# HandBrake/HandBrake

Measured on AMD Instinct MI355X. Metric: filtered frames/sec, 1080p YUV420p NLMeans+decomb chain, higher is better.
Workload: dtype u8 (f32 NLMeans weights, 16-bit fixed-point scaler as zimg, sharpen mix = the reference's f64 expression, as one f32 multiply where init proves that equal); 1 GPU; BASELINE configs[3]: decomb(31, EEDI2 bob) -> nlmeans medium -> cropscale lanczos 1920x1080 -> 3840x2160 -> lapsharp, 1080i YUV420P 8-bit in, inputs resident in HBM; input=1920x1080, output=3840x2160, streams_per_gpu=1, content=interlaced, stream_frames=48, stage_streams=2, parallelism=1 GPU(s) x 1 independent stream(s), device=AMD Radeon Graphics (gfx950:sramecc+:xnack-, 256 CUs)

## Files before the change

### handbrake_amd/csrc/eedi2.hip

```cpp
#include "eedi2_vote.h"
#include "eedi2_engine.h"

#include <atomic>
#include <algorithm>

namespace {

constexpr int PEAK = 255, NEUTRAL = 128;
constexpr int EEDI_MAX_FIELDS = EEDI_MAX_BATCH;
constexpr size_t GUARD = 32768;

__constant__ uint8_t c_limlut[33] = { 6, 6, 7, 7, 8, 8, 9, 9, 9, 10, 10, 11, 11, 12, 12, 12, 12, 12, 12, 12,
                                      12, 12, 12, 12, 12, 12, 12, 12, 12, 12, 12, 255, 255 };

constexpr int LIM_N = 33, LIM_PAD = 40;
__device__ __forceinline__ void lim_fill(uint8_t *tab, int tid)
{
    if (tid < LIM_N) tab[tid] = c_limlut[tid];
}

struct P3
{
    uint8_t *a[3];
    uint8_t *b[3];
    uint8_t *c[3];
    uint8_t *d[3];
    uint8_t *e[3];
    uint8_t *f[3];
    uint8_t *g[3];
    int pitch[3], width[3], height[3];
    size_t   fstride;
    uint32_t tffbits;
    const uint32_t *pflags;
    uint32_t pepoch;
};

struct PL { uint8_t *a, *b, *c, *d, *e, *f, *g; };
__device__ __forceinline__ PL plane_ptrs(const P3 &P, int pl, size_t off)
{
    PL q = { P.a[pl] + off, P.b[pl] + off, P.c[pl] + off, P.d[pl], P.e[pl] + off, P.f[pl] + off, P.g[pl] + off };
    if (q.d) q.d += off;
    return q;
}
#define FIELD_PLANE(P)                                                      \
    const int fld = (int)blockIdx.z / 3, pl = (int)blockIdx.z - 3 * fld;    \
    const int tff = (int)(((P).tffbits >> fld) & 1u);                       \
    const PL Q = plane_ptrs((P), pl, (size_t)fld * (P).fstride);            \
     \
     \
    const bool maskless = (P).pflags[blockIdx.z] != (P).pepoch;             \
    (void)tff; (void)maskless

__device__ __forceinline__ int iabs(int v) { return v < 0 ? -v : v; }
__device__ __forceinline__ int hbhip_align_up_dev(int v, int a) { return (v + a - 1) / a * a; }

__device__ __forceinline__ int wave_list_slots(int *counter, unsigned n)
{
    const uint64_t b0 = __ballot(n & 1u), b1 = __ballot(n & 2u), b2 = __ballot(n & 4u);
    const int total = __popcll(b0) + 2 * __popcll(b1) + 4 * __popcll(b2);
    auto below = [](uint64_t m) { return (int)__builtin_amdgcn_mbcnt_hi((uint32_t)(m >> 32), __builtin_amdgcn_mbcnt_lo((uint32_t)m, 0u)); };
    int base = 0;
    if (total)
    {
        if ((threadIdx.x & 63) == 0) base = atomicAdd(counter, total);
        base = __builtin_amdgcn_readfirstlane(base);
    }
    return base + below(b0) + 2 * below(b1) + 4 * below(b2);
}

__device__ __forceinline__ int sad3(const uint8_t *a, int ai, const uint8_t *b, int bi)
{
    return iabs((int)a[ai - 1] - (int)b[bi - 1]) + iabs((int)a[ai] - (int)b[bi]) + iabs((int)a[ai + 1] - (int)b[bi + 1]);
}

__device__ __forceinline__ int sorted_mid(int *v, int n)
{
    for (int i = 1; i < n; i++)
    {
        const int t = v[i];
        int j = i;
        while (j > 0 && v[j - 1] > t) { v[j] = v[j - 1]; j--; }
        v[j] = t;
    }
    return (n & 1) ? v[n >> 1] : (v[(n - 1) >> 1] + v[n >> 1] + 1) >> 1;
}


constexpr int ABSENT = 1000;

__device__ __forceinline__ void cswap(int &a, int &b)
{
    const int lo = min(a, b), hi = max(a, b);
    a = lo; b = hi;
}

__device__ __forceinline__ int mid9(int &v0, int &v1, int &v2, int &v3, int &v4, int &v5, int &v6, int &v7, int &v8, int n)
{
    cswap(v0, v3); cswap(v1, v7); cswap(v2, v5); cswap(v4, v8);
    cswap(v0, v7); cswap(v2, v4); cswap(v3, v8); cswap(v5, v6);
    cswap(v0, v2); cswap(v1, v3); cswap(v4, v5); cswap(v7, v8);
    cswap(v1, v4); cswap(v3, v6); cswap(v5, v7);
    cswap(v0, v1); cswap(v2, v4); cswap(v3, v5); cswap(v6, v8);
    cswap(v2, v3); cswap(v4, v5); cswap(v6, v7);
    cswap(v1, v2); cswap(v3, v4); cswap(v5, v6);
    const bool n5 = n <= 5, n7 = n <= 7;
    const int hi = n5 ? v2 : (n7 ? v3 : v4);
    const int lo = n5 ? v1 : (n7 ? v2 : v3);
    return (n & 1) ? hi : (lo + hi + 1) >> 1;
}

__device__ __forceinline__ int mid6(int &v0, int &v1, int &v2, int &v3, int &v4, int &v5, int n)
{
    cswap(v0, v5); cswap(v1, v3); cswap(v2, v4);
    cswap(v1, v2); cswap(v3, v4);
    cswap(v0, v3); cswap(v2, v5);
    cswap(v0, v1); cswap(v2, v3); cswap(v4, v5);
    cswap(v1, v2); cswap(v3, v4);
    const int lo = n <= 4 ? v1 : v2;
    const int hi = n <= 3 ? v1 : (n <= 5 ? v2 : v3);
    return (n & 1) ? hi : (lo + hi + 1) >> 1;
}

__device__ __forceinline__ void vote1(int v, int mid, int lim, int &sum, int &cnt)
{
    const bool in = (int)__builtin_amdgcn_sad_u16((uint32_t)v, (uint32_t)mid, 0u) <= lim;
    cnt += in;
    sum += in ? v : 0;
}

#define XY_PLANE(P)                                                         \
    FIELD_PLANE(P);                                                         \
    const int x = blockIdx.x * blockDim.x + threadIdx.x;                    \
    const int y = blockIdx.y * blockDim.y + threadIdx.y;                    \
    const int pitch = (P).pitch[pl], width = (P).width[pl], height = (P).height[pl]; \
    (void)width; (void)height; (void)pitch

struct Win12 { uint32_t w0, w1, w2; };

__device__ __forceinline__ Win12 ldwin(const uint8_t *row_at_x)
{
    const uint32_t *p = reinterpret_cast<const uint32_t *>(row_at_x);
    return Win12{p[-1], p[0], p[1]};
}

__device__ __forceinline__ int wb(const Win12 &w, int i)
{
    const int k = i + 4;
    const uint32_t d = k < 4 ? w.w0 : (k < 8 ? w.w1 : w.w2);
    return (int)((d >> (8 * (k & 3))) & 0xffu);
}

__device__ __forceinline__ void st4(uint8_t *dst_at_x, const int (&out)[4], int x, int limit)
{
// ... 367 lines not shown
        if (!(y == 1 || mp[x - 1 + u] == PEAK || mp[x + u] == PEAK || mp[x + 1 + u] == PEAK)) continue;
        if (!(y == height - 2 || mn[x - 1 - u] == PEAK || mn[x - u] == PEAK || mn[x + 1 - u] == PEAK)) continue;
        const int diffsn = sad3(sc, x, sn, x - u);
        const int diffsp = sad3(sc, x, sp, x + u);
        const int diffps = sad3(sp, x, sc, x - u);
        const int diffns = sad3(sn, x, sc, x + u);
        const int diff = diffsn + diffsp + diffps + diffns;
        int diffd = diffsp + diffns, diffe = diffsn + diffps;
        if (diff < minb) { dirb = u; minb = diff; }
        if (y > 1)
        {
            const int diff2pp = sad3(s2p, x, sp, x - u);
            const int diffp2p = sad3(sp, x, s2p, x + u);
            const int diffa = diff + diff2pp + diffp2p;
            diffd += diffp2p;
            diffe += diff2pp;
            if (diffa < mina) { dira = u; mina = diffa; }
        }
        if (y < height - 2)
        {
            const int diff2nn = sad3(s2n, x, sn, x + u);
            const int diffn2n = sad3(sn, x, s2n, x - u);
            const int diffc = diff + diff2nn + diffn2n;
            diffd += diff2nn;
            diffe += diffn2n;
            if (diffc < minc) { dirc = u; minc = diffc; }
        }
        if (diffd < mind) { dird = u; mind = diffd; }
        if (diffe < mine) { dire = u; mine = diffe; }
    }
    int order[5], k = 0;
    if (dira != -5000) order[k++] = dira;
    if (dirb != -5000) order[k++] = dirb;
    if (dirc != -5000) order[k++] = dirc;
    if (dird != -5000) order[k++] = dird;
    if (dire != -5000) order[k++] = dire;
    int out = NEUTRAL;
    if (k > 1)
    {
        const int mid = sorted_mid(order, k);
        const int tlim = max((int)c_limlut[iabs(mid)] >> 2, 2);
        int sum = 0, cnt = 0;
        for (int i = 0; i < k; i++)
            if (iabs(order[i] - mid) <= tlim) { cnt++; sum += order[i]; }
        if (cnt > 1) out = (NEUTRAL + ((int)((float)sum / (float)cnt) * 4)) & 0xff;
    }
    Q.c[(size_t)y * pitch + x] = (uint8_t)out;
}

#ifdef HBHIP_DEV_STATS
__device__ unsigned long long g_cd_stats[24];
#define CD_STAT(i, v) atomicAdd(&g_cd_stats[i], (unsigned long long)(v))
#else
#define CD_STAT(i, v) ((void)0)
#endif
constexpr int CD_W = 256, CD_HALO = 32, CD_LW = CD_W + 2 * CD_HALO;



__device__ __forceinline__ int calc_dir_vote(int ta, int tb, int tc, int td, int te)
{
    constexpr int BIG = 1 << 20;
    int v0 = ta ? ta - 32 : BIG, v1 = tb ? tb - 32 : BIG, v2 = tc ? tc - 32 : BIG, v3 = td ? td - 32 : BIG, v4 = te ? te - 32 : BIG;
    const int k = (ta != 0) + (tb != 0) + (tc != 0) + (td != 0) + (te != 0);
#define CD_CX(a, b) { const int lo_ = min(a, b), hi_ = max(a, b); a = lo_; b = hi_; }
    CD_CX(v0, v1) CD_CX(v3, v4) CD_CX(v2, v4) CD_CX(v2, v3) CD_CX(v0, v3) CD_CX(v0, v2) CD_CX(v1, v4) CD_CX(v1, v3) CD_CX(v1, v2)
#undef CD_CX
    int out = NEUTRAL;
    if (k > 1)
    {
        const int lo = k == 2 ? v0 : (k == 5 ? v2 : v1);
        const int hi = k >= 4 ? v2 : v1;
        const int mid = (lo + hi + 1) >> 1;
        static_assert(CD_HALO - 2 <= 30, "the closed form of limlut covers entries 0..30");
        const int tlim = iabs(mid) >= 13 ? 3 : 2;
        int sum = 0, cnt = 0;
        if (iabs(v0 - mid) <= tlim) { cnt++; sum += v0; }
        if (iabs(v1 - mid) <= tlim) { cnt++; sum += v1; }
        if (iabs(v2 - mid) <= tlim) { cnt++; sum += v2; }
        if (iabs(v3 - mid) <= tlim) { cnt++; sum += v3; }
        if (iabs(v4 - mid) <= tlim) { cnt++; sum += v4; }
        if (cnt > 1) out = (NEUTRAL + ((int)((float)sum / (float)cnt) * 4)) & 0xff;
    }
    return out;
}

template <bool EDGE, typename PASS>
__device__ __forceinline__ int calc_dir_search(const uint32_t *tr, PASS pass, int maxdt, bool first, bool last, int nt13, int nt19)
{
    const uint32_t F2p = tr[0], Fp = tr[CD_LW], Fc = tr[2 * CD_LW], Fn = tr[3 * CD_LW], F2n = tr[4 * CD_LW];
    const int ctr = (int)((Fc >> 8) & 0xff);
    const int vert = iabs(ctr - (int)((Fn >> 8) & 0xff)) + iabs(ctr - (int)((Fp >> 8) & 0xff));
    uint32_t kb = (uint32_t)min(nt13, vert * 6) << 16, ka = (uint32_t)min(nt19, vert * 9) << 16;
    uint32_t kc = ka, kd = kb, ke = kb;
    typedef __attribute__((address_space(3))) const uint32_t *lds_u32;
    uint32_t ap0 = (uint32_t)(uintptr_t)(lds_u32)(tr - maxdt), am0 = (uint32_t)(uintptr_t)(lds_u32)(tr + maxdt);
    uint32_t tag0 = (uint32_t)(32 - maxdt);
    asm volatile("" : "+v"(ap0), "+v"(am0), "+s"(tag0));
#define SADH(a, b, acc) __builtin_amdgcn_sad_hi_u8((a), (b), (acc))
    while (pass)
    {
        const int jj = sizeof(PASS) == 8 ? __ffsll((unsigned long long)pass) - 1 : __ffs((unsigned int)pass) - 1;
        pass &= pass - (PASS)1;
        const uint32_t tag = (uint32_t)jj + tag0;
        const lds_u32 tp = (lds_u32)(uintptr_t)(ap0 + 4u * (uint32_t)jj), tm = (lds_u32)(uintptr_t)(am0 - 4u * (uint32_t)jj);
        const uint32_t e1 = SADH(Fp, tm[2 * CD_LW], SADH(Fc, tm[3 * CD_LW], 0u));
        const uint32_t d1 = SADH(Fn, tp[2 * CD_LW], SADH(Fc, tp[1 * CD_LW], tag));
        const uint32_t diff = e1 + d1;
        uint32_t diffd = d1, diffe = e1;
        kb = min(kb, diff);
        if (!EDGE || !first)
        {
            const uint32_t diff2pp = SADH(F2p, tm[1 * CD_LW], tag);
            const uint32_t diffp2p = SADH(Fp, tp[0 * CD_LW], 0u);
            diffd += diffp2p;
            diffe += diff2pp;
            ka = min(ka, diff + diff2pp + diffp2p);
        }
        else
            diffe += tag;
        if (!EDGE || !last)
        {
            const uint32_t diff2nn = SADH(F2n, tp[3 * CD_LW], 0u);
            const uint32_t diffn2n = SADH(Fn, tm[4 * CD_LW], 0u);
            diffd += diff2nn;
            diffe += diffn2n;
            kc = min(kc, diff + diff2nn + diffn2n);
        }
        kd = min(kd, diffd);
        ke = min(ke, diffe);
    }
#undef SADH
    return calc_dir_vote((int)((ka & 0xffffu) >> 1), (int)(kb & 0xffffu), (int)(kc & 0xffffu), (int)(kd & 0xffffu), (int)(ke & 0xffffu));
}

template <int R, bool PRED>
__device__ __forceinline__ void calc_dir_dense(const uint32_t *tr, int maxdt, const uint32_t (&up)[R], const uint32_t (&dn)[R],
                                               int nt13, int nt19, uint32_t (&ka)[R], uint32_t (&kb)[R], uint32_t (&kc)[R],
                                               uint32_t (&kd)[R], uint32_t (&ke)[R])
{
    constexpr int NS = R + 4, NE = R + 3;
#define SADH(a, b, acc) __builtin_amdgcn_sad_hi_u8((a), (b), (acc))
    uint32_t T[NS];
#pragma unroll
    for (int r = 0; r < NS; r++) T[r] = tr[r * CD_LW];
#pragma unroll
    for (int j = 0; j < R; j++)
    {
        const int ctr = (int)((T[j + 2] >> 8) & 0xff);
        const int vert = iabs(ctr - (int)((T[j + 3] >> 8) & 0xff)) + iabs(ctr - (int)((T[j + 1] >> 8) & 0xff));
        kb[j] = (uint32_t)min(nt13, vert * 6) << 16; ka[j] = (uint32_t)min(nt19, vert * 9) << 16;
        kc[j] = ka[j]; kd[j] = kb[j]; ke[j] = kb[j];
    }
    auto sums = [&](const uint32_t (&Pv)[NE], const uint32_t (&Qv)[NE], const uint32_t (&X)[R], uint32_t (&ca)[R], uint32_t (&cb)[R],
                    uint32_t (&cc)[R], uint32_t (&cd)[R], uint32_t (&ce)[R]) {
        uint32_t S[NE], P2[NE - 1], Q2[NE - 1];
#pragma unroll
        for (int r = 0; r < NE; r++) S[r] = Pv[r] + Qv[r];
#pragma unroll
        for (int r = 0; r < NE - 1; r++) { P2[r] = Pv[r] + Pv[r + 1]; Q2[r] = Qv[r] + Qv[r + 1]; }
        if (PRED)
        {
#pragma unroll
            for (int j = 0; j < R; j++)
            {
                cb[j] = S[j + 1] + S[j + 2] + X[j]; ca[j] = cb[j] + S[j]; cc[j] = cb[j] + S[j + 3];
                ce[j] = P2[j] + P2[j + 2] + X[j];   cd[j] = Q2[j] + Q2[j + 2] + X[j];
            }
        }
        else
        {
            uint32_t S2[NE - 1], S3[NE - 2];
#pragma unroll
            for (int r = 0; r < NE - 1; r++) S2[r] = S[r] + S[r + 1];
#pragma unroll
            for (int r = 0; r < NE - 2; r++) S3[r] = S2[r] + S[r + 2];
#pragma unroll
            for (int j = 0; j < R; j++)
            {
                cb[j] = S2[j + 1]; ca[j] = S3[j]; cc[j] = S3[j + 1];
                ce[j] = P2[j] + P2[j + 2]; cd[j] = Q2[j] + Q2[j + 2];
            }
        }
    };
    uint32_t X1[R], X2[R];
#pragma unroll
    for (int j = 0; j < R; j++) { X1[j] = 0; X2[j] = 0; }
    {
        uint32_t Pv[NE], ca[R], cb[R], cc[R], cd[R], ce[R];
#pragma unroll
        for (int r = 0; r < NE; r++) Pv[r] = SADH(T[r], T[r + 1], 32u);
        if (PRED)
        {
#pragma unroll
            for (int j = 0; j < R; j++) X1[j] = (up[j] << 30) & 0x40000000u;
        }
        sums(Pv, Pv, X1, ca, cb, cc, cd, ce);
#pragma unroll
        for (int j = 0; j < R; j++)
        {
            ka[j] = min(ka[j], ca[j]); kb[j] = min(kb[j], cb[j]); kc[j] = min(kc[j], cc[j]);
            kd[j] = min(kd[j], cd[j]); ke[j] = min(ke[j], ce[j]);
        }
    }
    for (int d = 1; d <= maxdt; d++)
    {
        const uint32_t *tp = tr + d, *tm = tr - d;
        uint32_t Pl[NS], Mi[NS];
#pragma unroll
        for (int r = 0; r < NS; r++) { Pl[r] = tp[r * CD_LW]; Mi[r] = tm[r * CD_LW]; }
        const uint32_t t1 = 32u + (uint32_t)d, t2 = 32u - (uint32_t)d;
        uint32_t P1[NE], Q1[NE], Pn[NE], Qn[NE];
#pragma unroll
        for (int r = 0; r < NE; r++)
        {
            P1[r] = SADH(T[r], Mi[r + 1], t1); Q1[r] = SADH(Pl[r], T[r + 1], t1);
            Pn[r] = SADH(T[r], Pl[r + 1], t2); Qn[r] = SADH(Mi[r], T[r + 1], t2);
        }
        if (PRED)
        {
            const uint32_t sh = 30u - (uint32_t)d;
#pragma unroll
            for (int j = 0; j < R; j++) { X1[j] = (up[j] << sh) & 0x40000000u; X2[j] = (dn[j] << sh) & 0x40000000u; }
        }
#ifdef CD_SEQ
        (void)P1; (void)Q1; (void)Pn; (void)Qn;
        {
            uint32_t Pa[NE], Qa[NE], ca[R], cb[R], cc[R], cd[R], ce[R];
#pragma unroll
            for (int r = 0; r < NE; r++) { Pa[r] = SADH(T[r], Mi[r + 1], t1); Qa[r] = SADH(Pl[r], T[r + 1], t1); }
            if (PRED)
            {
                const uint32_t sh = 30u - (uint32_t)d;
#pragma unroll
                for (int j = 0; j < R; j++) X1[j] = (up[j] << sh) & 0x40000000u;
            }
            sums(Pa, Qa, X1, ca, cb, cc, cd, ce);
#pragma unroll
            for (int j = 0; j < R; j++)
            {
                ka[j] = min(ka[j], ca[j]); kb[j] = min(kb[j], cb[j]); kc[j] = min(kc[j], cc[j]);
                kd[j] = min(kd[j], cd[j]); ke[j] = min(ke[j], ce[j]);
            }
        }
#pragma unroll
        for (int j = 0; j < R; j++) asm volatile("" : "+v"(ka[j]), "+v"(kb[j]), "+v"(kc[j]), "+v"(kd[j]), "+v"(ke[j]));
        __builtin_amdgcn_sched_barrier(0);
        {
            uint32_t Pa[NE], Qa[NE], ca[R], cb[R], cc[R], cd[R], ce[R];
#pragma unroll
            for (int r = 0; r < NE; r++) { Pa[r] = SADH(T[r], Pl[r + 1], t2); Qa[r] = SADH(Mi[r], T[r + 1], t2); }
            if (PRED)
            {
                const uint32_t sh = 30u - (uint32_t)d;
#pragma unroll
                for (int j = 0; j < R; j++) X2[j] = (dn[j] << sh) & 0x40000000u;
            }
            sums(Pa, Qa, X2, ca, cb, cc, cd, ce);
#pragma unroll
            for (int j = 0; j < R; j++)
            {
                ka[j] = min(ka[j], ca[j]); kb[j] = min(kb[j], cb[j]); kc[j] = min(kc[j], cc[j]);
                kd[j] = min(kd[j], cd[j]); ke[j] = min(ke[j], ce[j]);
            }
        }
        continue;
#endif
        uint32_t ca[R], cb[R], cc[R], cd[R], ce[R], na[R], nb[R], nc[R], nd[R], ne[R];
        sums(P1, Q1, X1, ca, cb, cc, cd, ce);
        sums(Pn, Qn, X2, na, nb, nc, nd, ne);
#pragma unroll
        for (int j = 0; j < R; j++)
        {
            ka[j] = min(ka[j], min(ca[j], na[j])); kb[j] = min(kb[j], min(cb[j], nb[j])); kc[j] = min(kc[j], min(cc[j], nc[j]));
            kd[j] = min(kd[j], min(cd[j], nd[j])); ke[j] = min(ke[j], min(ce[j], ne[j]));
        }
    }
#undef SADH
}

__device__ __forceinline__ uint64_t calc_dir_window(const uint64_t *bits, int start, uint64_t lenmask)
{
    const int wq = start >> 6, sh = start & 63;
    const uint64_t lo = bits[wq], hi = bits[wq + 1];
    const uint64_t w = sh ? (lo >> sh) | (hi << (64 - sh)) : lo;
    return (w | (w >> 1) | (w >> 2)) & lenmask;
}

#ifndef CD_WAVES_ATTR
#define CD_WAVES_ATTR
#endif
template <int R>
__global__ __launch_bounds__(CD_W) CD_WAVES_ATTR void k_calc_dir_rows(P3 P, int maxd, int nt13, int nt19, int dense_min, uint32_t padv)
{
    constexpr int NS = R + 4, NM = R + 2, RW = CD_LW / 4, RQ = CD_LW / 16;
    __shared__ __attribute__((aligned(16))) uint8_t s_band[NS + NM][CD_LW];
    __shared__ __attribute__((aligned(16))) uint32_t s_tri[NS][CD_LW];
    __shared__ uint64_t s_bits[NM][8];
    __shared__ uint16_t s_list[R * CD_W];
    __shared__ __attribute__((aligned(16))) uint8_t s_out[R][CD_W];
    __shared__ int s_count;
    FIELD_PLANE(P);
    const int pitch = P.pitch[pl], width = P.width[pl], height = P.height[pl];
    const int x0 = blockIdx.x * CD_W, y0 = blockIdx.y * R;
    if (y0 >= height || x0 >= pitch) return;
    const int tid = threadIdx.x, lane = tid & 63;
    if (maskless)
    {
#pragma unroll
        for (int jr = 0; jr < R; jr += CD_W / 64)
        {
            const int j = jr + (tid >> 6), y = y0 + j, xb = x0 + 4 * lane;
            if (j < R && y < height && xb < pitch) *reinterpret_cast<uint32_t *>(Q.c + (size_t)y * pitch + xb) = pad_bytes(0xffffffffu, xb, width, padv);
        }
        return;
    }
    if (tid == 0) s_count = 0;
    if (tid < NM * 3) s_bits[tid / 3][5 + tid % 3] = 0;
    uint32_t *band = reinterpret_cast<uint32_t *>(&s_band[0][0]);
    {
        const uint8_t *sb = Q.b + x0 - CD_HALO, *mb = Q.a + x0 - CD_HALO;
        for (int i = tid; i < (NS + NM) * RQ; i += CD_W)
        {
            const int r = i / RQ, c16 = i - r * RQ;
            const uint8_t *src = r < NS ? sb + (ptrdiff_t)min(y0 - 2 + r, height + 1) * pitch
                                        : mb + (ptrdiff_t)min(y0 - 1 + (r - NS), height) * pitch;
            reinterpret_cast<uint4 *>(band)[i] = reinterpret_cast<const uint4 *>(src)[c16];
        }
    }
    __syncthreads();
#pragma unroll
    for (int jr = 0; jr < R; jr += CD_W / 64)
    {
        const int j = jr + (tid >> 6), y = y0 + j, xb = x0 + 4 * lane;
        if (R % (CD_W / 64) != 0 && j >= R) break;
        const uint32_t *mrow = band + (NS + j + 1) * RW + CD_HALO / 4 + lane;
        const uint32_t prev = mrow[-1], cur = mrow[0], next = mrow[1];
        auto eq255 = [](uint32_t v) { return (((v & 0x7f7f7f7fu) + 0x01010101u) & v) & 0x80808080u; };
        uint32_t act = eq255(cur) & (eq255(__builtin_amdgcn_alignbyte(cur, prev, 3)) | eq255(__builtin_amdgcn_alignbyte(next, cur, 1)));
        if (y < 1 || y >= height - 1) act = 0;
#pragma unroll
        for (int k = 0; k < 4; k++)
            if (xb + k < 1 || xb + k >= width - 1) act &= ~(0x80u << (8 * k));
        reinterpret_cast<uint32_t *>(&s_out[j][0])[lane] = 0xffffffffu;
        int total = 0, before = 0;
#pragma unroll
        for (int k = 0; k < 4; k++)
        {
            const uint64_t bal = __ballot((act >> (8 * k + 7)) & 1u);
            before += (int)__builtin_amdgcn_mbcnt_hi((uint32_t)(bal >> 32), __builtin_amdgcn_mbcnt_lo((uint32_t)bal, 0u));
            total += __popcll(bal);
        }
        int base = 0;
        if (lane == 0 && total) base = atomicAdd(&s_count, total);
        base = __builtin_amdgcn_readfirstlane(base) + before;
#pragma unroll
        for (int k = 0; k < 4; k++)
            if ((act >> (8 * k + 7)) & 1u) s_list[base++] = (uint16_t)((j << 8) | (4 * lane + k));
    }
    __syncthreads();
    const int count = s_count;
    const int maxdt = pl == 0 ? maxd : (maxd >> 1);
    const int len = 2 * maxdt + 1;
    const uint64_t lenmask = (1ull << len) - 1ull;
    const bool edge = y0 <= 1 || y0 + R - 1 >= height - 2;
    const bool dense = R >= 4 && !edge && count >= dense_min;
    if (count)
    {
        for (int i = tid; i < NS * RW; i += CD_W)
        {
            const uint32_t d0 = band[i], d1 = band[i + 1];
            reinterpret_cast<uint4 *>(&s_tri[0][0])[i] =
                make_uint4(d0 & 0x00ffffffu, __builtin_amdgcn_alignbyte(d1, d0, 1) & 0x00ffffffu,
                           __builtin_amdgcn_alignbyte(d1, d0, 2) & 0x00ffffffu, __builtin_amdgcn_alignbyte(d1, d0, 3) & 0x00ffffffu);
        }
        for (int k = 0; k < 2; k++)
        {
            if (k == 1 && tid >= 64) break;
            const int i = tid + k * CD_W;
    #pragma unroll
            for (int m = 0; m < NM; m++)
            {
                const uint64_t w = __ballot(s_band[NS + m][i] == PEAK);
                if (lane == 0) s_bits[m][i >> 6] = w;
            }
        }
        __syncthreads();
    }
#ifdef HBHIP_DEV_STATS
    if (tid == 0) { CD_STAT(0, 1); CD_STAT(1, count != 0); CD_STAT(2, count); CD_STAT(7, dense); }
#endif
    if (R >= 4 && dense)
    {
        constexpr int RD = R >= 4 ? R : 1;
        const int lx = tid, px = x0 + lx, b = lx + CD_HALO - 1;
        const int startu = max(-px + 1, -maxdt), stopu = min(width - 2 - px, maxdt);
        uint64_t range = 0;
        if (stopu >= startu)
        {
            const int nb = stopu - startu + 1;
            range = (nb >= 64 ? ~0ull : ((1ull << nb) - 1ull)) << (startu + maxdt);
        }
        uint64_t win[RD + 2];
#pragma unroll
        for (int m = 0; m < RD + 2; m++) win[m] = calc_dir_window(s_bits[m], b - maxdt, lenmask);
        uint32_t up[RD], dn[RD], act = 0, inactive = 0;
#pragma unroll
        for (int j = 0; j < RD; j++)
        {
            const uint8_t *mr = &s_band[NS + j + 1][CD_HALO + lx];
            const bool a = px >= 1 && px < width - 1 && mr[0] == PEAK && (mr[-1] == PEAK || mr[1] == PEAK);
            const uint64_t pass = a ? range & win[j] & (__brevll(win[j + 2]) >> (64 - len)) : 0ull;
            const uint64_t npass = ~pass;
            up[j] = (uint32_t)(npass >> maxdt);
            dn[j] = __brev((uint32_t)npass << (31 - maxdt));
            act |= (uint32_t)a << j;
            inactive |= (up[j] | dn[j]) & ((2u << maxdt) - 1u);
        }
        if (__any(act != 0))
        {
            uint32_t ka[RD], kb[RD], kc[RD], kd[RD], ke[RD];
            const uint32_t *tr = &s_tri[0][b];
            if (__all(inactive == 0)) calc_dir_dense<RD, false>(tr, maxdt, up, dn, nt13, nt19, ka, kb, kc, kd, ke);
            else                      calc_dir_dense<RD, true>(tr, maxdt, up, dn, nt13, nt19, ka, kb, kc, kd, ke);
#pragma unroll
            for (int j = 0; j < RD; j++)
                if ((act >> j) & 1u)
                    s_out[j][lx] = (uint8_t)calc_dir_vote((int)((ka[j] & 0xffffu) / 6u), (int)((kb[j] & 0xffffu) >> 2), (int)((kc[j] & 0xffffu) / 6u),
                                                          (int)((kd[j] & 0xffffu) >> 2), (int)((ke[j] & 0xffffu) >> 2));
#ifdef HBHIP_DEV_STATS
            if (lane == 0) { CD_STAT(8, 1); CD_STAT(9, __all(inactive == 0)); }
#endif
        }
        __syncthreads();
    }
    else if (count)
    {
        for (int p = tid; p < count; p += CD_W)
        {
            const uint32_t id = s_list[p];
            const int j = (int)(id >> 8), lx = (int)(id & 255u), y = y0 + j, px = x0 + lx, b = lx + CD_HALO - 1;
            const int startu = max(-px + 1, -maxdt), stopu = min(width - 2 - px, maxdt);
            uint64_t pass = 0;
            if (stopu >= startu)
            {
                const int nb = stopu - startu + 1;
                pass = (nb >= 64 ? ~0ull : ((1ull << nb) - 1ull)) << (startu + maxdt);
                if (y != 1)          pass &= calc_dir_window(s_bits[j], b - maxdt, lenmask);
                if (y != height - 2) pass &= __brevll(calc_dir_window(s_bits[j + 2], b - maxdt, lenmask)) >> (64 - len);
            }
#ifdef HBHIP_DEV_STATS
            {
                int n = __popcll(pass), mx = n, sm = n, ln = 1;
                for (int o = 32; o; o >>= 1) { mx = max(mx, __shfl_xor(mx, o)); sm += __shfl_xor(sm, o); ln += __shfl_xor(ln, o); }
                const uint64_t act = __ballot(1);
                if (lane == __ffsll((unsigned long long)act) - 1) { CD_STAT(3, 1); CD_STAT(4, sm); CD_STAT(5, mx); CD_STAT(6, ln); }
            }
#endif
            const uint32_t *tr = &s_tri[j][b];
            int out;
            if (len <= 32)
                out = edge ? calc_dir_search<true, uint32_t>(tr, (uint32_t)pass, maxdt, y == 1, y == height - 2, nt13, nt19)
                           : calc_dir_search<false, uint32_t>(tr, (uint32_t)pass, maxdt, false, false, nt13, nt19);
            else
                out = edge ? calc_dir_search<true, uint64_t>(tr, pass, maxdt, y == 1, y == height - 2, nt13, nt19)
                           : calc_dir_search<false, uint64_t>(tr, pass, maxdt, false, false, nt13, nt19);
            s_out[j][lx] = (uint8_t)out;
        }
        __syncthreads();
    }
#pragma unroll
    for (int jr = 0; jr < R; jr += CD_W / 64)
    {
        const int j = jr + (tid >> 6), y = y0 + j, xb = x0 + 4 * lane;
        if (j < R && y < height && xb < pitch)
            *reinterpret_cast<uint32_t *>(Q.c + (size_t)y * pitch + xb) = pad_bytes(reinterpret_cast<const uint32_t *>(&s_out[j][0])[lane], xb, width, padv);
    }
}


__device__ __forceinline__ int dir_map_px(int u0, int u1, int u2, int c0, int c1, int c2, int n0, int n1, int n2,
                                          bool up_ok, bool dn_ok, int expand, const uint8_t *limlut)
{
    const bool h0 = up_ok && u0 != PEAK, h1 = up_ok && u1 != PEAK, h2 = up_ok && u2 != PEAK;
    const bool h3 = c0 != PEAK, h4 = !expand && c1 != PEAK, h5 = c2 != PEAK;
    const bool h6 = dn_ok && n0 != PEAK, h7 = dn_ok && n1 != PEAK, h8 = dn_ok && n2 != PEAK;
    const int u = h0 + h1 + h2 + h3 + h4 + h5 + h6 + h7 + h8;
    if (u < (expand ? 5 : 4)) return expand ? c1 : PEAK;
    int v0 = h0 ? u0 : ABSENT, v1 = h1 ? u1 : ABSENT, v2 = h2 ? u2 : ABSENT;
    int v3 = h3 ? c0 : ABSENT, v4 = h4 ? c1 : ABSENT, v5 = h5 ? c2 : ABSENT;
    int v6 = h6 ? n0 : ABSENT, v7 = h7 ? n1 : ABSENT, v8 = h8 ? n2 : ABSENT;
    int s0 = v0, s1 = v1, s2 = v2, s3 = v3, s4 = v4, s5 = v5, s6 = v6, s7 = v7, s8 = v8;
    const int mid = mid9(s0, s1, s2, s3, s4, s5, s6, s7, s8, u);
    const int lim = limlut[iabs(mid - NEUTRAL) >> 2];
    int sum = 0, count = 0;
    vote1(v0, mid, lim, sum, count); vote1(v1, mid, lim, sum, count); vote1(v2, mid, lim, sum, count);
    vote1(v3, mid, lim, sum, count); vote1(v4, mid, lim, sum, count); vote1(v5, mid, lim, sum, count);
    vote1(v6, mid, lim, sum, count); vote1(v7, mid, lim, sum, count); vote1(v8, mid, lim, sum, count);
    const int val = vote_avg(sum + mid, count + 1);
    if (expand) return count >= 5 ? (val & 0xff) : c1;
    if (count < 4 || (count < 5 && c1 == PEAK)) return PEAK;
    return val & 0xff;
}

__device__ __forceinline__ uint32_t ff_bytes(uint32_t v)
{
    return (((v & 0x7f7f7f7fu) + 0x01010101u) & v) & 0x80808080u;
}

typedef uint16_t u16x2 __attribute__((ext_vector_type(2)));
typedef int16_t i16x2 __attribute__((ext_vector_type(2)));
constexpr uint32_t PK_ABSENT_HI = 0x7f00u;
__device__ __forceinline__ u16x2 pk(uint32_t v) { return __builtin_bit_cast(u16x2, v); }
__device__ __forceinline__ uint32_t un(u16x2 v) { return __builtin_bit_cast(uint32_t, v); }
__device__ __forceinline__ u16x2 pk1(uint32_t both) { return pk(both * 0x00010001u); }
__device__ __forceinline__ u16x2 pk_lt(u16x2 a, u16x2 b) { return (u16x2)((u16x2)(a - b) >> 15); }
__device__ __forceinline__ void cswap2(u16x2 &a, u16x2 &b)
{
    const u16x2 lo = __builtin_elementwise_min(a, b), hi = __builtin_elementwise_max(a, b);
    a = lo; b = hi;
}
__device__ __forceinline__ u16x2 limlut2(u16x2 i)
{
    const u16x2 g = pk_lt(pk1(7), i);
    const u16x2 l = __builtin_elementwise_min((u16x2)(((i - g) >> 1) + pk1(6)), pk1(12));
    const u16x2 big = pk_lt(pk1(30), i) * pk1(255);
    return __builtin_elementwise_max(l, big);
}
#define PK_BYTES(hi, lo, a, b) __builtin_amdgcn_perm((hi), (lo), 0x0c000c00u | ((uint32_t)(b) << 16) | (uint32_t)(a))

template <int K>
__device__ __forceinline__ uint32_t dir_map_pair(const Win12 &wu, const Win12 &wc, const Win12 &wd, int expand)
{
    u16x2 v[9];
    {
        const Win12 *rows[3] = { &wu, &wc, &wd };
#pragma unroll
        for (int r = 0; r < 3; r++)
        {
            const uint32_t w0 = rows[r]->w0, w1 = rows[r]->w1, w2 = rows[r]->w2;
            if (K == 0)
            {
                v[3 * r + 0] = pk(PK_BYTES(w1, w0, 3, 4));
                v[3 * r + 1] = pk(PK_BYTES(w1, w0, 4, 5));
                v[3 * r + 2] = pk(PK_BYTES(w1, w0, 5, 6));
            }
            else
            {
                v[3 * r + 0] = pk(PK_BYTES(w1, w0, 5, 6));
                v[3 * r + 1] = pk(PK_BYTES(w1, w0, 6, 7));
                v[3 * r + 2] = pk(PK_BYTES(w2, w1, 3, 4));
            }
        }
    }
    const u16x2 c1 = v[4];
    u16x2 a[9];
    uint32_t absent = 0;
#pragma unroll
    for (int i = 0; i < 9; i++)
    {
        a[i] = (u16x2)((v[i] + pk1(1)) >> 8);
        absent += un(a[i]);
        v[i] = v[i] + a[i] * pk1(PK_ABSENT_HI);
    }
    u16x2 s0 = v[0], s1 = v[1], s2 = v[2], s3 = v[3], s4 = v[4], s5 = v[5], s6 = v[6], s7 = v[7], s8 = v[8];
    cswap2(s0, s3); cswap2(s1, s7); cswap2(s2, s5); cswap2(s4, s8);
    cswap2(s0, s7); cswap2(s2, s4); cswap2(s3, s8); cswap2(s5, s6);
    cswap2(s0, s2); cswap2(s1, s3); cswap2(s4, s5); cswap2(s7, s8);
    cswap2(s1, s4); cswap2(s3, s6); cswap2(s5, s7);
    cswap2(s0, s1); cswap2(s2, s4); cswap2(s3, s5); cswap2(s6, s8);
    cswap2(s2, s3); cswap2(s4, s5); cswap2(s6, s7);
    cswap2(s1, s2); cswap2(s3, s4); cswap2(s5, s6);
    const u16x2 ab = pk(absent), one = pk1(1), zero = pk1(0);
    const uint32_t m5 = un(zero - pk_lt(pk1(3), ab));
    const uint32_t m7 = un(zero - pk_lt(one, ab));
    const uint32_t modd = un((ab & one) - one);
#define PK_SEL(m, x, y) (((m) & (x)) | (~(m) & (y)))
    const uint32_t hi = PK_SEL(m5, un(s2), PK_SEL(m7, un(s3), un(s4)));
    const uint32_t lo = PK_SEL(m5, un(s1), PK_SEL(m7, un(s2), un(s3)));
    const u16x2 mid = pk(PK_SEL(modd, hi, un((u16x2)((pk(lo) + pk(hi) + one) >> 1))));
    const i16x2 t = __builtin_bit_cast(i16x2, (u16x2)(mid - pk1(NEUTRAL)));
    const u16x2 lim1 = limlut2(__builtin_bit_cast(u16x2, __builtin_elementwise_max(t, (i16x2)(-t))) >> 2) + one;
// ... 2072 lines not shown
```

Measured before the change: 9129 output frames/s.

## Stream EEDI2 calc_dir dense SAD sums row-by-row and split predicated path

Restructures the dense direction search so SAD partial sums are produced and consumed incrementally per row via a rolling CdRun helper, loading shifted rows on the fly instead of materialising whole Pl/Mi/P/Q arrays. Keys are fenced per row to bound live ranges. The predicated path is split into two half-height calls when the row count is at least 8. The aim is to cut VGPR pressure and spills in the calc_dir kernel, at the cost of reloading the centre rows twice in the split path and relying on the compiler to keep the rolling arrays in registers.

```diff
diff --git a/handbrake_amd/csrc/eedi2.hip b/handbrake_amd/csrc/eedi2.hip
--- a/handbrake_amd/csrc/eedi2.hip
+++ b/handbrake_amd/csrc/eedi2.hip
@@ -1,4 +1,5 @@
 #include "eedi2_vote.h"
+#include "eedi2_dense.h"
 #include "eedi2_engine.h"
 
 #include <atomic>
@@ -672,131 +673,67 @@
         kb[j] = (uint32_t)min(nt13, vert * 6) << 16; ka[j] = (uint32_t)min(nt19, vert * 9) << 16;
         kc[j] = ka[j]; kd[j] = kb[j]; ke[j] = kb[j];
     }
-    auto sums = [&](const uint32_t (&Pv)[NE], const uint32_t (&Qv)[NE], const uint32_t (&X)[R], uint32_t (&ca)[R], uint32_t (&cb)[R],
-                    uint32_t (&cc)[R], uint32_t (&cd)[R], uint32_t (&ce)[R]) {
-        uint32_t S[NE], P2[NE - 1], Q2[NE - 1];
-#pragma unroll
-        for (int r = 0; r < NE; r++) S[r] = Pv[r] + Qv[r];
-#pragma unroll
-        for (int r = 0; r < NE - 1; r++) { P2[r] = Pv[r] + Pv[r + 1]; Q2[r] = Qv[r] + Qv[r + 1]; }
-        if (PRED)
-        {
-#pragma unroll
-            for (int j = 0; j < R; j++)
-            {
-                cb[j] = S[j + 1] + S[j + 2] + X[j]; ca[j] = cb[j] + S[j]; cc[j] = cb[j] + S[j + 3];
-                ce[j] = P2[j] + P2[j + 2] + X[j];   cd[j] = Q2[j] + Q2[j + 2] + X[j];
-            }
-        }
-        else
-        {
-            uint32_t S2[NE - 1], S3[NE - 2];
-#pragma unroll
-            for (int r = 0; r < NE - 1; r++) S2[r] = S[r] + S[r + 1];
-#pragma unroll
-            for (int r = 0; r < NE - 2; r++) S3[r] = S2[r] + S[r + 2];
-#pragma unroll
-            for (int j = 0; j < R; j++)
-            {
-                cb[j] = S2[j + 1]; ca[j] = S3[j]; cc[j] = S3[j + 1];
-                ce[j] = P2[j] + P2[j + 2]; cd[j] = Q2[j] + Q2[j + 2];
-            }
-        }
-    };
-    uint32_t X1[R], X2[R];
-#pragma unroll
-    for (int j = 0; j < R; j++) { X1[j] = 0; X2[j] = 0; }
-    {
-        uint32_t Pv[NE], ca[R], cb[R], cc[R], cd[R], ce[R];
-#pragma unroll
-        for (int r = 0; r < NE; r++) Pv[r] = SADH(T[r], T[r + 1], 32u);
-        if (PRED)
-        {
-#pragma unroll
-            for (int j = 0; j < R; j++) X1[j] = (up[j] << 30) & 0x40000000u;
-        }
-        sums(Pv, Pv, X1, ca, cb, cc, cd, ce);
-#pragma unroll
-        for (int j = 0; j < R; j++)
-        {
-            ka[j] = min(ka[j], ca[j]); kb[j] = min(kb[j], cb[j]); kc[j] = min(kc[j], cc[j]);
-            kd[j] = min(kd[j], cd[j]); ke[j] = min(ke[j], ce[j]);
+    {
+        CdRun<R, PRED> run;
+#pragma unroll
+        for (int r = 0; r < NE; r++)
+        {
+            const uint32_t Pv = SADH(T[r], T[r + 1], 32u);
+            run.push(r, Pv, Pv);
+            if (r >= 3)
+            {
+                const int j = r - 3;
+                const uint32_t X = PRED ? (up[j] << 30) & 0x40000000u : 0u;
+                uint32_t ca, cb, cc, cd, ce;
+                run.cands(j, X, ca, cb, cc, cd, ce);
+                ka[j] = min(ka[j], ca); kb[j] = min(kb[j], cb); kc[j] = min(kc[j], cc); kd[j] = min(kd[j], cd); ke[j] = min(ke[j], ce);
+                CD_FENCE_KEYS(j);
+            }
         }
     }
     for (int d = 1; d <= maxdt; d++)
     {
         const uint32_t *tp = tr + d, *tm = tr - d;
-        uint32_t Pl[NS], Mi[NS];
-#pragma unroll
-        for (int r = 0; r < NS; r++) { Pl[r] = tp[r * CD_LW]; Mi[r] = tm[r * CD_LW]; }
-        const uint32_t t1 = 32u + (uint32_t)d, t2 = 32u - (uint32_t)d;
-        uint32_t P1[NE], Q1[NE], Pn[NE], Qn[NE];
+        const uint32_t t1 = 32u + (uint32_t)d, t2 = 32u - (uint32_t)d, sh = 30u - (uint32_t)d;
+        CdRun<R, PRED> pos, neg;
+        uint32_t Pl0 = tp[0], Mi0 = tm[0], Pl1 = tp[CD_LW], Mi1 = tm[CD_LW];
 #pragma unroll
         for (int r = 0; r < NE; r++)
         {
-            P1[r] = SADH(T[r], Mi[r + 1], t1); Q1[r] = SADH(Pl[r], T[r + 1], t1);
-            Pn[r] = SADH(T[r], Pl[r + 1], t2); Qn[r] = SADH(Mi[r], T[r + 1], t2);
-        }
-        if (PRED)
-        {
-            const uint32_t sh = 30u - (uint32_t)d;
-#pragma unroll
-            for (int j = 0; j < R; j++) { X1[j] = (up[j] << sh) & 0x40000000u; X2[j] = (dn[j] << sh) & 0x40000000u; }
-        }
-#ifdef CD_SEQ
-        (void)P1; (void)Q1; (void)Pn; (void)Qn;
-        {
-            uint32_t Pa[NE], Qa[NE], ca[R], cb[R], cc[R], cd[R], ce[R];
-#pragma unroll
-            for (int r = 0; r < NE; r++) { Pa[r] = SADH(T[r], Mi[r + 1], t1); Qa[r] = SADH(Pl[r], T[r + 1], t1); }
-            if (PRED)
-            {
-                const uint32_t sh = 30u - (uint32_t)d;
-#pragma unroll
-                for (int j = 0; j < R; j++) X1[j] = (up[j] << sh) & 0x40000000u;
-            }
-            sums(Pa, Qa, X1, ca, cb, cc, cd, ce);
-#pragma unroll
-            for (int j = 0; j < R; j++)
-            {
-                ka[j] = min(ka[j], ca[j]); kb[j] = min(kb[j], cb[j]); kc[j] = min(kc[j], cc[j]);
-                kd[j] = min(kd[j], cd[j]); ke[j] = min(ke[j], ce[j]);
-            }
-        }
-#pragma unroll
-        for (int j = 0; j < R; j++) asm volatile("" : "+v"(ka[j]), "+v"(kb[j]), "+v"(kc[j]), "+v"(kd[j]), "+v"(ke[j]));
-        __builtin_amdgcn_sched_barrier(0);
-        {
-            uint32_t Pa[NE], Qa[NE], ca[R], cb[R], cc[R], cd[R], ce[R];
-#pragma unroll
-            for (int r = 0; r < NE; r++) { Pa[r] = SADH(T[r], Pl[r + 1], t2); Qa[r] = SADH(Mi[r], T[r + 1], t2); }
-            if (PRED)
-            {
-                const uint32_t sh = 30u - (uint32_t)d;
-#pragma unroll
-                for (int j = 0; j < R; j++) X2[j] = (dn[j] << sh) & 0x40000000u;
-            }
-            sums(Pa, Qa, X2, ca, cb, cc, cd, ce);
-#pragma unroll
-            for (int j = 0; j < R; j++)
-            {
-                ka[j] = min(ka[j], ca[j]); kb[j] = min(kb[j], cb[j]); kc[j] = min(kc[j], cc[j]);
-                kd[j] = min(kd[j], cd[j]); ke[j] = min(ke[j], ce[j]);
-            }
-        }
-        continue;
-#endif
-        uint32_t ca[R], cb[R], cc[R], cd[R], ce[R], na[R], nb[R], nc[R], nd[R], ne[R];
-        sums(P1, Q1, X1, ca, cb, cc, cd, ce);
-        sums(Pn, Qn, X2, na, nb, nc, nd, ne);
-#pragma unroll
-        for (int j = 0; j < R; j++)
-        {
-            ka[j] = min(ka[j], min(ca[j], na[j])); kb[j] = min(kb[j], min(cb[j], nb[j])); kc[j] = min(kc[j], min(cc[j], nc[j]));
-            kd[j] = min(kd[j], min(cd[j], nd[j])); ke[j] = min(ke[j], min(ce[j], ne[j]));
+            uint32_t Pl2 = 0, Mi2 = 0;
+            if (r + 2 < NS) { Pl2 = tp[(r + 2) * CD_LW]; Mi2 = tm[(r + 2) * CD_LW]; }
+            pos.push(r, SADH(T[r], Mi1, t1), SADH(Pl0, T[r + 1], t1));
+            neg.push(r, SADH(T[r], Pl1, t2), SADH(Mi0, T[r + 1], t2));
+            Pl0 = Pl1; Mi0 = Mi1; Pl1 = Pl2; Mi1 = Mi2;
+            if (r >= 3)
+            {
+                const int j = r - 3;
+                const uint32_t X1 = PRED ? (up[j] << sh) & 0x40000000u : 0u, X2 = PRED ? (dn[j] << sh) & 0x40000000u : 0u;
+                uint32_t ca, cb, cc, cd, ce, na, nb, nc, nd, ne;
+                pos.cands(j, X1, ca, cb, cc, cd, ce);
+                neg.cands(j, X2, na, nb, nc, nd, ne);
+                ka[j] = min(ka[j], min(ca, na)); kb[j] = min(kb[j], min(cb, nb)); kc[j] = min(kc[j], min(cc, nc));
+                kd[j] = min(kd[j], min(cd, nd)); ke[j] = min(ke[j], min(ce, ne));
+                CD_FENCE_KEYS(j);
+            }
         }
     }
 #undef SADH
+}
+
+template <int N, bool PRED, int RD, int J0>
+__device__ __forceinline__ void calc_dir_dense_vote(const uint32_t *tr, int maxdt, const uint32_t (&up)[RD], const uint32_t (&dn)[RD],
+                                                    uint32_t act, int nt13, int nt19, uint8_t *out)
+{
+    uint32_t u[N], v[N], ka[N], kb[N], kc[N], kd[N], ke[N];
+#pragma unroll
+    for (int j = 0; j < N; j++) { u[j] = up[J0 + j]; v[j] = dn[J0 + j]; }
+    calc_dir_dense<N, PRED>(tr + J0 * CD_LW, maxdt, u, v, nt13, nt19, ka, kb, kc, kd, ke);
+#pragma unroll
+    for (int j = 0; j < N; j++)
+        if ((act >> (J0 + j)) & 1u)
+            out[(J0 + j) * CD_W] = (uint8_t)calc_dir_vote((int)((ka[j] & 0xffffu) / 6u), (int)((kb[j] & 0xffffu) >> 2), (int)((kc[j] & 0xffffu) / 6u),
+                                                          (int)((kd[j] & 0xffffu) >> 2), (int)((ke[j] & 0xffffu) >> 2));
 }
 
 __device__ __forceinline__ uint64_t calc_dir_window(const uint64_t *bits, int start, uint64_t lenmask)
@@ -939,15 +876,15 @@
         }
         if (__any(act != 0))
         {
-            uint32_t ka[RD], kb[RD], kc[RD], kd[RD], ke[RD];
             const uint32_t *tr = &s_tri[0][b];
-            if (__all(inactive == 0)) calc_dir_dense<RD, false>(tr, maxdt, up, dn, nt13, nt19, ka, kb, kc, kd, ke);
-            else                      calc_dir_dense<RD, true>(tr, maxdt, up, dn, nt13, nt19, ka, kb, kc, kd, ke);
-#pragma unroll
-            for (int j = 0; j < RD; j++)
-                if ((act >> j) & 1u)
-                    s_out[j][lx] = (uint8_t)calc_dir_vote((int)((ka[j] & 0xffffu) / 6u), (int)((kb[j] & 0xffffu) >> 2), (int)((kc[j] & 0xffffu) / 6u),
-                                                          (int)((kd[j] & 0xffffu) >> 2), (int)((ke[j] & 0xffffu) >> 2));
+            if (__all(inactive == 0))
+                calc_dir_dense_vote<RD, false, RD, 0>(tr, maxdt, up, dn, act, nt13, nt19, &s_out[0][lx]);
+            else
+            {
+                constexpr int RH = RD >= 8 ? RD / 2 : RD;
+                calc_dir_dense_vote<RH, true, RD, 0>(tr, maxdt, up, dn, act, nt13, nt19, &s_out[0][lx]);
+                if constexpr (RH < RD) calc_dir_dense_vote<RD - RH, true, RD, RH>(tr, maxdt, up, dn, act, nt13, nt19, &s_out[0][lx]);
+            }
 #ifdef HBHIP_DEV_STATS
             if (lane == 0) { CD_STAT(8, 1); CD_STAT(9, __all(inactive == 0)); }
 #endif
diff --git a/handbrake_amd/csrc/eedi2_dense.h b/handbrake_amd/csrc/eedi2_dense.h
--- /dev/null
+++ b/handbrake_amd/csrc/eedi2_dense.h
@@ -0,0 +1,32 @@
+#pragma once
+#include <hip/hip_runtime.h>
+#include <cstdint>
+
+template <int R, bool PRED>
+struct CdRun
+{
+    static constexpr int NE = R + 3;
+    uint32_t P[NE], Q[NE], S[NE], P2[NE], Q2[NE], S2[NE], S3[NE];
+    __device__ __forceinline__ void push(int r, uint32_t p, uint32_t q)
+    {
+        P[r] = p; Q[r] = q; S[r] = p + q;
+        if (r >= 1) { P2[r - 1] = P[r - 1] + p; Q2[r - 1] = Q[r - 1] + q; }
+        if (!PRED && r >= 1) S2[r - 1] = S[r - 1] + S[r];
+        if (!PRED && r >= 2) S3[r - 2] = S2[r - 2] + S[r];
+    }
+    __device__ __forceinline__ void cands(int j, uint32_t X, uint32_t &ca, uint32_t &cb, uint32_t &cc, uint32_t &cd, uint32_t &ce) const
+    {
+        if (PRED)
+        {
+            cb = S[j + 1] + S[j + 2] + X; ca = cb + S[j]; cc = cb + S[j + 3];
+            ce = P2[j] + P2[j + 2] + X;   cd = Q2[j] + Q2[j + 2] + X;
+        }
+        else
+        {
+            cb = S2[j + 1]; ca = S3[j]; cc = S3[j + 1];
+            ce = P2[j] + P2[j + 2]; cd = Q2[j] + Q2[j + 2];
+        }
+    }
+};
+
+#define CD_FENCE_KEYS(j) asm volatile("" : "+v"(ka[j]), "+v"(kb[j]), "+v"(kc[j]), "+v"(kd[j]), "+v"(ke[j]))
```

New measurement: 9294 output frames/s, median of 6. 1.8% higher.
